# donglinb/ORB-SLAM-BIRDVIEW

Hardware: AMD Instinct MI355X
Metric: ORB features/sec per GPU (1280×720, 2000 kp, 8 levels) + Hamming matches/sec (higher is better)
Workload: dtype u8; 1 GPU; C3 1280x720 KITTI-style synthetic, 2000 features, 8 levels; width=1280, height=720, nfeatures=2000, nlevels=8, ini_th_fast=20, min_th_fast=7, batch_per_gpu=256, global_batch=256, parallelism=frame-sharded x1 (no collective), batches_in_flight=2

## Files before the change

### orb-slam-birdview_amd/csrc/extract_kernels.hip

```cpp
#include "glibc_trig.h"
#include "orbgpu_internal.h"
#include "pattern31_data.inc"

#include <algorithm>
#include <cstring>

namespace orbgpu {

__constant__ __attribute__((aligned(16))) int8_t c_pattern[1024] = {ORBGPU_PATTERN31_VALUES};
__constant__ __attribute__((aligned(16))) float c_pattern_f[1024] = {ORBGPU_PATTERN31_VALUES};

struct IcMaskTable {
    uint32_t m[64][4];
};
constexpr IcMaskTable make_ic_masks() {
    IcMaskTable t{};
    constexpr int umax[16] = {15, 15, 15, 15, 14, 14, 14, 13, 13, 12, 11, 10, 9, 8, 6, 3};
    for (int l = 0; l < 64; l++) {
        const int r = (l >> 1) < 30 ? (l >> 1) : 30, v = r - 15, h = l & 1;
        const int d = umax[v < 0 ? -v : v];
        for (int i = 0; i < 4; i++) {
            uint32_t m = 0;
            for (int j = 0; j < 4; j++) {
                const int u = 4 * (4 * h + i) + j;
// ... 1799 lines not shown
                               err, par, ost);
    else
        octree_level<false, NT, CP>(g, L, f, l, smem, C, keys, knodeAll + o, lvlKps, lvlCount, err, par, ost);
}


template <int NT>
__global__ __launch_bounds__(NT) void k_octree(const Geom* __restrict__ g,
                                                           const uint32_t* __restrict__ cands,
                                                           const uint32_t* __restrict__ candFirst,
                                                           uint32_t* __restrict__ keysAll,
                                                           uint16_t* __restrict__ knodeAll,
                                                           uint32_t* __restrict__ lvlKps, int* __restrict__ lvlCount,
                                                           int* __restrict__ err, int lds_keys,
                                                           unsigned long long* __restrict__ ostamps, int lbase) {
    extern __shared__ __attribute__((aligned(16))) int smem[];
    octree_task<NT, 0>(g, blockIdx.x, lbase + (int)blockIdx.y, smem, cands, candFirst, keysAll, knodeAll, lvlKps,
                       lvlCount, err, lds_keys, ostamps);
}

constexpr float kAtanScale = (float)(180 / 3.14159265358979323846);
constexpr float kP1 = 0.9997878412794807f * kAtanScale;
constexpr float kP3 = -0.3258083974640975f * kAtanScale;
constexpr float kP5 = 0.1555786518463281f * kAtanScale;
constexpr float kP7 = -0.04432655554792128f * kAtanScale;
constexpr float kFactorPI = (float)(3.14159265358979323846 / 180.f);

__device__ __forceinline__ float fast_atan2(float y, float x) {
    const float ax = fabsf(x), ay = fabsf(y);
    float a, c, c2;
    if (ax >= ay) {
        c = ay / (ax + (float)2.220446049250313e-16);
        c2 = c * c;
        a = (((kP7 * c2 + kP5) * c2 + kP3) * c2 + kP1) * c;
    } else {
        c = ax / (ay + (float)2.220446049250313e-16);
        c2 = c * c;
        a = 90.f - (((kP7 * c2 + kP5) * c2 + kP3) * c2 + kP1) * c;
    }
    if (x < 0) a = 180.f - a;
    if (y < 0) a = 360.f - a;
    return a;
}



constexpr int kDescRtCols = 37, kDescWinOff = 2976, kDescWaveBytes = kDescWinOff + kDescWin * kDescWinPitch;
constexpr bool desc_overlap_ok() {
    return 2 * kRtPitch * kDescRtCols <= kDescWinOff + 6 * kDescWinPitch && kDescWinOff % 16 == 0 &&
           kDescWaveBytes % 16 == 0 && 4 * kDescWaveBytes + 256 <= 160 * 1024 / 8;
}
static_assert(desc_overlap_ok(), "k_describe LDS overlap");

struct DescSlot {
    bool ok, interior;
    int s, l, x, y, score, outIdx;
    LevelPtr src;
};

template <int CP = 0>
__device__ __forceinline__ DescSlot desc_slot(const Geom* __restrict__ g, int f, int s, const int* cnts,
                                              const uint32_t* __restrict__ lvlKps, const uint8_t* frames,
                                              long long framePitch, int rowStride, const uint8_t* pyr) {
    DescSlot d;
    d.s = s;
    d.ok = false;
    d.interior = false;
    if (s >= g->nkpcap) return d;
    const int nl = g->nlevels;
    int l = 0;
    while (l + 1 < nl && s >= g->L[l + 1].kp_base) ++l;
    const LevelGeom& L = g->L[l];
    const int k = s - L.kp_base;
    auto cnt = [&](int i) -> int {
        if constexpr (CP != 0) return __hip_atomic_load(&cnts[i], __ATOMIC_RELAXED, __HIP_MEMORY_SCOPE_AGENT);
        else return cnts[i];
    };
    if (k >= cnt(l)) return d;
    int outIdx = k;
    for (int i = 0; i < l; i++) outIdx += cnt(i);
    uint32_t kp;
    if constexpr (CP != 0) kp = __hip_atomic_load(&lvlKps[(long long)f * g->nkpcap + s], __ATOMIC_RELAXED, __HIP_MEMORY_SCOPE_AGENT);
    else kp = lvlKps[(long long)f * g->nkpcap + s];
    d.ok = true;
    d.l = l;
    d.x = kp & 0xFFF;
    d.y = (kp >> 12) & 0xFFF;
    d.score = kp >> 24;
    d.outIdx = outIdx;
    d.src = level_ptr(g, l, frames, framePitch, rowStride, pyr, f);
    const bool aligned = ((reinterpret_cast<uintptr_t>(d.src.p) | (uintptr_t)d.src.stride) & 3) == 0;
    d.interior = aligned && d.x >= 21 && d.x + 27 <= L.w && d.y >= 21 && d.y + 21 < L.h;
    return d;
}

template <int CP = 0>
__device__ __forceinline__ void desc_issue(const DescSlot& d, int lane, uint32_t (&v)[9]) {
    const int a0 = (d.x - 21) & ~3;
    const int stride = __builtin_amdgcn_readfirstlane(d.src.stride);
    const uint64_t rb = reinterpret_cast<uint64_t>(d.src.p + (long long)(d.y - 21) * stride + a0);
    const uint64_t rbu = ((uint64_t)(uint32_t)__builtin_amdgcn_readfirstlane((unsigned)(rb >> 32)) << 32) |
                         (uint64_t)(uint32_t)__builtin_amdgcn_readfirstlane((unsigned)rb);
    const auto rsrc = __builtin_amdgcn_make_buffer_rsrc(reinterpret_cast<void*>(rbu), 0, (kDescWin - 1) * stride + 48,
                                                          0x00020000);
    const int wy0 = (int)(__umul24((unsigned)lane, 2731u) >> 15), ww = lane - wy0 * 12;
    const int off = (int)roi_off(wy0, stride, 4 * ww);
#pragma unroll
    for (int r = 0; r < 8; r++) v[r] = __builtin_amdgcn_raw_buffer_load_b32(rsrc, off, 5 * r * stride, CP);
    v[8] = __builtin_amdgcn_raw_buffer_load_b32(rsrc, lane < 36 ? off : 0x40000000, 40 * stride, CP);
}

template <bool ALLEVEN, bool FMA>
__device__ __forceinline__ void brief_sampled(const uint16_t* rt, float a, float b, const float (&pf)[4][4], int colBase,
                                              int xsimd, ushort2_t K01, ushort2_t K23, ushort2_t K45, ushort2_t K60,
                                              int lane, unsigned long long* __restrict__ dst) {
    typedef const uint32_t __attribute__((address_space(3))) lds_u32;
    constexpr uint32_t kC = (uint32_t)kRtPitch * 0x400000u + 0x4B400000u;
    static_assert((kC & 1u) == 0, "the element bias must keep the parity");
    const uint32_t lbase = (uint32_t)(uintptr_t)(lds_u32*)reinterpret_cast<const uint32_t*>(rt) - 2u * kC;
    const uint32_t xlim = (uint32_t)(xsimd - colBase) + 0x4B400000u;
    const uint32_t bias = sgpr_const(32767u);
    typedef float f32x2_t __attribute__((ext_vector_type(2)));
    const f32x2_t ab = {a, b}, nba = {-b, a}, cr = {12582930.0f, 12582930.0f};
    auto sample = [&](f32x2_t pp) -> uint32_t {
        const f32x2_t pyv = __builtin_shufflevector(pp, pp, 1, 1), pxv = __builtin_shufflevector(pp, pp, 0, 0);
        const f32x2_t t = pyv * nba;
        const f32x2_t r = (FMA ? __builtin_elementwise_fma(pxv, ab, t) : pxv * ab + t) + cr;
        const float fx = r.x, fy = r.y;
        const uint32_t xbits = __builtin_bit_cast(uint32_t, fx);
        const uint32_t ybits = __builtin_bit_cast(uint32_t, fy);
        const uint32_t idx = __umul24(xbits, (unsigned)kRtPitch) + ybits;
        uint32_t ie = idx & ~1u;
        asm("" : "+v"(ie));
        lds_u32* rp = (lds_u32*)(uintptr_t)(lbase + (ie << 1));
        const uint32_t sh = idx << 4;
        const uint32_t d0 = rp[0], d1 = rp[1], d2 = rp[2], d3 = rp[3];
        uint32_t S = __builtin_amdgcn_udot2(K01, __builtin_bit_cast(ushort2_t, __builtin_amdgcn_alignbit(d1, d0, sh)), 0u, false);
        S = __builtin_amdgcn_udot2(K23, __builtin_bit_cast(ushort2_t, __builtin_amdgcn_alignbit(d2, d1, sh)), S, false);
        S = __builtin_amdgcn_udot2(K45, __builtin_bit_cast(ushort2_t, __builtin_amdgcn_alignbit(d3, d2, sh)), S, false);
        S = __builtin_amdgcn_udot2(K60, __builtin_bit_cast(ushort2_t, __builtin_amdgcn_alignbit(d3, d3, sh)), S, false);
        if (ALLEVEN) return S + bias + ((S >> 16) & 1u);
        return S + (xbits < xlim ? bias + ((S >> 16) & 1u) : 32768u);
    };
    unsigned long long mq[4];
#pragma unroll
    for (int gq = 0; gq < 4; gq++) {
        const uint32_t r0 = sample(f32x2_t{pf[gq][0], pf[gq][1]});
        const uint32_t r1 = sample(f32x2_t{pf[gq][2], pf[gq][3]});
        mq[gq] = __ballot((r0 >> 16) < min(r1 >> 16, 255u));
    }
    if (lane < 4) dst[lane] = lane == 0 ? mq[0] : lane == 1 ? mq[1] : lane == 2 ? mq[2] : mq[3];
}

template <bool FMA, int CP = 0>
__device__ __forceinline__ void desc_body(const Geom* __restrict__ g, const DescSlot& d, int f, int lane,
                                          const uint32_t (&v)[9], uint8_t* wbase, uint16_t* rt,
                                          orb_keypoint* __restrict__ outK, uint8_t* __restrict__ outD, int kpCap,
                                          unsigned long long* __restrict__ dstamps) {
    const int l = d.l, x = d.x, y = d.y, score = d.score, outIdx = d.outIdx;
    const LevelGeom& L = g->L[l];
    const LevelPtr src = d.src;
    [[maybe_unused]] unsigned long long* dst_st = dstamps ? dstamps + ((long long)f * g->nkpcap + d.s) * 8 : nullptr;
#if ORBGPU_KERNEL_STAMPS
#define DESC_STAMP(k) \
    if (dst_st && lane == 0) dst_st[(k)] = __builtin_amdgcn_s_memtime();
#else
#define DESC_STAMP(k)
#endif
    DESC_STAMP(0);
    const uint4 mm = reinterpret_cast<const uint4*>(&c_ic_masks.m[0][0])[lane];
    const uint32_t icm[4] = {mm.x, mm.y, mm.z, mm.w};
    uint32_t* w32 = reinterpret_cast<uint32_t*>(wbase);
    int sh;
    if (d.interior) {
#pragma unroll
        for (int r = 0; r < 9; r++)
            if (r < 8 || lane < 36) w32[lane + 60 * r] = v[r];
        sh = (x - 21) & 3;
    } else {
#pragma unroll
        for (int hb = 0; hb < 2; hb++) {
            uint8_t v[15];
#pragma unroll
            for (int r = 0; r < 15; r++) {
                const int idx = lane + 64 * (15 * hb + r);
                const int wy = (int)(__umul24((unsigned)idx, 24386u) >> 20), wx = idx - wy * kDescWin;
                int sy = y - 21 + wy, sx = x - 21 + wx;
                sy = sy < 0 ? -sy : (sy >= L.h ? 2 * L.h - 2 - sy : sy);
                sx = sx < 0 ? -sx : (sx >= L.w ? 2 * L.w - 2 - sx : sx);
                if constexpr (CP != 0) {
                    const auto brs = __builtin_amdgcn_make_buffer_rsrc(const_cast<uint8_t*>(src.p), 0, 0x7FFFFFFF, 0x00020000);
                    v[r] = idx < kDescWin * kDescWin ? __builtin_amdgcn_raw_buffer_load_b8(brs, (int)roi_off(sy, src.stride, sx), 0, CP)
                                                     : (uint8_t)0;
                } else {
                    v[r] = idx < kDescWin * kDescWin ? src.p[roi_off(sy, src.stride, sx)] : (uint8_t)0;
                }
            }
#pragma unroll
            for (int r = 0; r < 15; r++) {
                const int idx = lane + 64 * (15 * hb + r);
                const int wy = (int)(__umul24((unsigned)idx, 24386u) >> 20), wx = idx - wy * kDescWin;
                if (idx < kDescWin * kDescWin) wbase[wy * kDescWinPitch + wx] = v[r];
            }
        }
        sh = 0;
    }
    wave_lds_sync();
    DESC_STAMP(1);
#if defined(ORBGPU_DESC_CUT) && ORBGPU_DESC_CUT == 1
    if (lane == 0) outD[((long long)f * kpCap + outIdx) * 32] = wbase[lane];
    return;
#endif

    int m10 = 0, m01 = 0;
    if (lane < 62) {
        const int v = (lane >> 1) - 15, h = lane & 1;
        const int base = (21 + v) * kDescWinPitch + sh + 6;
        const int d0 = (base >> 2) + 4 * h, bs = base & 3;
        uint32_t w[5];
#pragma unroll
        for (int i = 0; i < 5; i++) w[i] = w32[d0 + i];
        const uint32_t wt0 = 0x04030201u + (uint32_t)h * 0x10101010u;
        uint32_t sI = 0, sW = 0;
#pragma unroll
        for (int i = 0; i < 4; i++) {
            const uint32_t bytes = __builtin_amdgcn_alignbyte(w[i + 1], w[i], bs) & icm[i];
            sI = __builtin_amdgcn_udot4(bytes, 0x01010101u, sI, false);
            sW = __builtin_amdgcn_udot4(bytes, wt0 + (uint32_t)i * 0x04040404u, sW, false);
        }
        m10 = (int)sW - 16 * (int)sI;
        m01 = v * (int)sI;
    }
    m10 = wave_sum(m10);
    m01 = wave_sum(m01);
    const float angle = fast_atan2((float)m01, (float)m10);
    DESC_STAMP(2);
#if defined(ORBGPU_DESC_CUT) && ORBGPU_DESC_CUT == 2
    if (lane == 0) outD[((long long)f * kpCap + outIdx) * 32] = (uint8_t)angle;
    return;
#endif

    {
        typedef int v4i_t __attribute__((ext_vector_type(4)));
        const int4* tp = g->desc_taps + sh * kDescTapTiles * 64 + lane;
        v4i_t bt[kDescTapTiles];
#pragma unroll
        for (int tc = 0; tc < kDescTapTiles; tc++) {
            const int4 q = tp[tc * 64];
            bt[tc] = v4i_t{q.x, q.y, q.z, q.w};
        }
        const int yl = lane & 15, kq = lane >> 4;
        const int bias = 128 * (g->gk[0] + g->gk[1] + g->gk[2] + g->gk[3] + g->gk[4] + g->gk[5] + g->gk[6]);
#pragma unroll
        for (int ty = 0; ty < 3; ty++) {
            const int y = min(16 * ty + yl, kDescWin - 1);
            const uint4 w = *reinterpret_cast<const uint4*>(wbase + y * kDescWinPitch + 16 * kq);
            const v4i_t a = v4i_t{(int)(w.x ^ 0x80808080u), (int)(w.y ^ 0x80808080u), (int)(w.z ^ 0x80808080u),
                                  (int)(w.w ^ 0x80808080u)};
            const int y0 = 16 * ty + 4 * kq;
#pragma unroll
            for (int tc = 0; tc < kDescTapTiles; tc++) {
                v4i_t d = v4i_t{bias, bias, bias, bias};
                d = __builtin_amdgcn_mfma_i32_16x16x64_i8(a, bt[tc], d, 0, 0, 0);
                const int c = 16 * tc + yl;
                if (y0 < kDescWin && c < kDescRtCols) {
                    uint2 pk;
                    pk.x = __builtin_amdgcn_perm((uint32_t)d[1], (uint32_t)d[0], 0x05040100u);
                    pk.y = __builtin_amdgcn_perm((uint32_t)d[3], (uint32_t)d[2], 0x05040100u);
                    *reinterpret_cast<uint2*>(rt + c * kRtPitch + y0) = pk;
                }
            }
        }
    }
    wave_lds_sync();
    DESC_STAMP(3);
#if defined(ORBGPU_DESC_CUT) && ORBGPU_DESC_CUT == 3
    if (lane == 0) outD[((long long)f * kpCap + outIdx) * 32] = (uint8_t)(angle + rt[lane]);
    return;
#endif

    const int xsimd = (g->variant & ORB_VARIANT_BLUR_HALFUP) ? 0 : (L.w & ~3);
    const int k0 = g->gk[0], k1 = g->gk[1], k2 = g->gk[2], k3 = g->gk[3], k4 = g->gk[4], k5 = g->gk[5],
              k6 = g->gk[6];
    const ushort2_t K01 = {(unsigned short)k0, (unsigned short)k1}, K23 = {(unsigned short)k2, (unsigned short)k3},
                    K45 = {(unsigned short)k4, (unsigned short)k5}, K60 = {(unsigned short)k6, 0};
    DESC_STAMP(4);

    float pf[4][4];
#pragma unroll
    for (int gq = 0; gq < 4; gq++) {
        const float4 pp = reinterpret_cast<const float4*>(c_pattern_f)[lane + 64 * gq];
        pf[gq][0] = pp.x;
        pf[gq][1] = pp.y;
        pf[gq][2] = pp.z;
        pf[gq][3] = pp.w;
    }
    const float ang = angle * kFactorPI;
    float a, b;
    glibc_sincosf(ang, &b, &a);
    DESC_STAMP(5);
    unsigned long long* dst = reinterpret_cast<unsigned long long*>(outD + ((long long)f * kpCap + outIdx) * 32);
    if (x + 18 < xsimd) brief_sampled<true, FMA>(rt, a, b, pf, x - 18, xsimd, K01, K23, K45, K60, lane, dst);
    else brief_sampled<false, FMA>(rt, a, b, pf, x - 18, xsimd, K01, K23, K45, K60, lane, dst);
    if (lane == 0) {
        orb_keypoint o;
        o.x = (float)x;
        o.y = (float)y;
        if (l != 0) {
            o.x *= L.scale;
            o.y *= L.scale;
        }
        o.size = L.patch_size;
        o.angle = angle;
        o.response = (float)score;
        o.octave = l;
        o.class_id = -1;
        outK[(long long)f * kpCap + outIdx] = o;
    }
    DESC_STAMP(6);
#undef DESC_STAMP
}

constexpr int kDescWaves = 4, kDescSlotsPerWave = 2;
template <bool FMA>
__global__ __launch_bounds__(256) __attribute__((amdgpu_waves_per_eu(8, 8))) void k_describe(const Geom* __restrict__ g, const uint8_t* __restrict__ frames,
                                                  long long framePitch, int rowStride, const uint8_t* __restrict__ pyr,
                                                  const uint32_t* __restrict__ lvlKps,
                                                  const int* __restrict__ lvlCount, orb_keypoint* __restrict__ outK,
                                                  uint8_t* __restrict__ outD, int* __restrict__ outN, int kpCap,
                                                  unsigned long long* __restrict__ dstamps, int spw,
                                                  const int* __restrict__ err, int* __restrict__ errHost) {
    __shared__ __attribute__((aligned(16))) uint8_t s_desc[kDescWaves * kDescWaveBytes + 256];
    uint8_t* const s_wave = s_desc + (size_t)__builtin_amdgcn_readfirstlane(threadIdx.x >> 6) * kDescWaveBytes;
    const int gx = (g->nkpcap + kDescWaves * spw - 1) / (kDescWaves * spw);
    const int nb = gridDim.x, q = nb >> 3, r = nb & 7, xcd = blockIdx.x & 7, j = blockIdx.x >> 3;
    const int lb = (xcd < r ? xcd * (q + 1) : r * (q + 1) + (xcd - r) * q) + j;
    const int f = lb / gx, bx = lb - f * gx;
    const int wv = __builtin_amdgcn_readfirstlane(threadIdx.x >> 6), lane = threadIdx.x & 63;
    const int nl = g->nlevels;
    const int* cnts = lvlCount + f * nl;
    const int s0 = (bx * kDescWaves + wv) * spw;
    auto write_n = [&]() {
        if (bx == 0 && threadIdx.x == 0) {
            int tot = 0;
            for (int i = 0; i < nl; i++) tot += cnts[i];
            outN[f] = tot;
            if (errHost && f == 0) *errHost = err[0] | err[1];
        }
    };
    if (s0 >= g->nkpcap) {
        write_n();
        return;
    }
    const DescSlot d0 = desc_slot(g, f, s0, cnts, lvlKps, frames, framePitch, rowStride, pyr);
    const DescSlot d1 = spw == 2 ? desc_slot(g, f, s0 + 1, cnts, lvlKps, frames, framePitch, rowStride, pyr)
                                 : DescSlot{};
    if (!d0.ok && !d1.ok) {
        write_n();
        return;
    }
    uint32_t v0[9], v1[9];
    if (d0.ok && d0.interior) desc_issue(d0, lane, v0);
    if (d1.ok && d1.interior) desc_issue(d1, lane, v1);
    write_n();
    if (d0.ok) desc_body<FMA>(g, d0, f, lane, v0, s_wave + kDescWinOff, reinterpret_cast<uint16_t*>(s_wave), outK, outD, kpCap, dstamps);
    if (d1.ok) {
        __builtin_amdgcn_sched_barrier(0);
        wave_lds_sync();
        desc_body<FMA>(g, d1, f, lane, v1, s_wave + kDescWinOff, reinterpret_cast<uint16_t*>(s_wave), outK, outD, kpCap, dstamps);
    }
}

__global__ __launch_bounds__(256) void k_upload_stream(const uint8_t* __restrict__ h_img, const uint32_t* h_flags,
                                                       uint32_t seq, uint8_t* __restrict__ d_img, int pitch, int h,
                                                       int band_rows, uint32_t* __restrict__ err) {
    __shared__ int s_ok;
    const int b = blockIdx.x;
    if (threadIdx.x == 0) {
        int ok = 0;
        for (int it = 0; it < (1 << 22); it++) {
            if (__hip_atomic_load(h_flags + b, __ATOMIC_RELAXED, __HIP_MEMORY_SCOPE_SYSTEM) == seq) {
                ok = 1;
                break;
            }
            __builtin_amdgcn_s_sleep(2);
        }
        if (!ok) *err = 1;
        s_ok = ok;
    }
    __syncthreads();
    if (!s_ok) return;
    __atomic_thread_fence(__ATOMIC_ACQUIRE);
    const int r0 = b * band_rows, r1 = min(h, r0 + band_rows);
    const size_t n16 = (size_t)(r1 - r0) * pitch / 16;
    const uint4* src = reinterpret_cast<const uint4*>(h_img + (size_t)r0 * pitch);
    uint4* dst = reinterpret_cast<uint4*>(d_img + (size_t)r0 * pitch);
    const size_t st = (size_t)gridDim.y * 256;
    for (size_t i = blockIdx.y * 256 + threadIdx.x; i < n16; i += 4 * st) {
        uint4 v[4];
#pragma unroll
        for (int u = 0; u < 4; u++)
            if (i + u * st < n16) v[u] = src[i + u * st];
#pragma unroll
        for (int u = 0; u < 4; u++)
            if (i + u * st < n16) dst[i + u * st] = v[u];
    }
}

hipError_t launch_upload_stream(const uint8_t* h_img, const uint32_t* h_flags, uint32_t seq, uint8_t* d_img, int pitch,
                                int h, int nbands, int band_rows, uint32_t* h_fail, hipStream_t stream) {
    hipLaunchKernelGGL(k_upload_stream, dim3(nbands, 4), dim3(256), 0, stream, h_img, h_flags, seq, d_img, pitch, h,
                       band_rows, h_fail);
    return hipGetLastError();
}

__global__ __launch_bounds__(256) void k_debug_sincosf(const float* __restrict__ x, int n, float* __restrict__ s,
                                                       float* __restrict__ c) {
    const int i = blockIdx.x * 256 + threadIdx.x;
    if (i >= n) return;
    float sv, cv;
    glibc_sincosf(x[i], &sv, &cv);
    s[i] = sv;
    c[i] = cv;
}

hipError_t launch_debug_sincosf(const float* d_x, int n, float* d_s, float* d_c, hipStream_t stream) {
    if (n <= 0) return hipSuccess;
    hipLaunchKernelGGL(k_debug_sincosf, dim3((n + 255) / 256), dim3(256), 0, stream, d_x, n, d_s, d_c);
    return hipGetLastError();
}


__device__ __forceinline__ int flow_ld(const int* p) { return __hip_atomic_load(p, __ATOMIC_RELAXED, __HIP_MEMORY_SCOPE_AGENT); }
__device__ __forceinline__ void flow_st(int* p, int v) { __hip_atomic_store(p, v, __ATOMIC_RELAXED, __HIP_MEMORY_SCOPE_AGENT); }
__device__ __forceinline__ int flow_add(int* p, int v) {
    return __hip_atomic_fetch_add(p, v, __ATOMIC_RELAXED, __HIP_MEMORY_SCOPE_AGENT);
}

template <int TQ>
__device__ __forceinline__ void flow_fast(const FlowArgs* __restrict__ Ap, int l, int f, int a, int b, int wv, int lane,
                                          uint8_t* smem) {
    if (wv >= b) return;
    const Geom* __restrict__ g = Ap->g;
    const int wb = g->fast_wave_bytes;
    uint16_t* tile = reinterpret_cast<uint16_t*>(smem + (size_t)wv * wb + 16);
    uint16_t* sList = reinterpret_cast<uint16_t*>(smem + (size_t)wv * wb + ((g->fast_rows * TQ * 2 + 32 + 15) & ~15));
    const int cell = g->L[l].cell_base + a + wv;
    const FastCellT c = fast_cell_t(g, Ap->cells, f * g->ncells + cell, Ap->frames, Ap->framePitch, Ap->rowStride,
                                    Ap->pyr, 0, g->ncells);
    uint32_t* candFirst = Ap->candFirst;
    int* cntOut = reinterpret_cast<int*>(candFirst + ((long long)c.f * g->ncells + c.cell) * kCandRec);
    if (!c.valid) {
        if (lane == 0) flow_st(cntOut, 0);
        return;
    }
    uint32_t v[8];
    if (c.aligned) fast_roi_issue<kCpSc1>(c, lane, v);
    fast_roi_store<TQ, kCpSc1>(c, lane, v, tile);
    fast_cell_body<TQ, kCpSc1>(g, c, lane, tile, sList, Ap->cands, candFirst, cntOut, nullptr, 0);
}

__device__ __forceinline__ void flow_resize(const FlowArgs* __restrict__ Ap, int l, int f, int a, int b, int tid,
                                            uint8_t* smem) {
    const Geom* __restrict__ g = Ap->g;
    const int q = tid >> 8;
    const int th = (g->L[l].rs_tiled & 2) ? 32 : 16;
    const int gxl = (g->L[l].w + kRsTileW - 1) / kRsTileW;
    const int tile = a + q;
    const int by = tile / gxl, bx = tile - by * gxl;
    const int rq = Ap->rsQuarter;
    uint8_t* qb = smem + (size_t)q * rq;
    int4* scx = reinterpret_cast<int4*>(qb + rq - (kRsTileW + 32) * 16);
    int4* scy = scx + kRsTileW;
    const ResizeCoef* cf = Ap->rcoef + Ap->roff.o[l];
    const bool on = q < b;
    const bool gen = (g->variant & ORB_VARIANT_RESIZE_GENERIC) != 0;
    const uint8_t* frames = Ap->frames;
    const long long fp = Ap->framePitch;
    const int rs = Ap->rowStride;
    uint8_t* pyr = Ap->pyr;
    if (th == 32) {
        if (gen) resize_tile<32, true, kCpSc1>(g, cf, l, frames, fp, rs, pyr, f, bx, by, tid & 255, qb, scx, scy, on);
        else resize_tile<32, false, kCpSc1>(g, cf, l, frames, fp, rs, pyr, f, bx, by, tid & 255, qb, scx, scy, on);
    } else {
        if (gen) resize_tile<16, true, kCpSc1>(g, cf, l, frames, fp, rs, pyr, f, bx, by, tid & 255, qb, scx, scy, on);
        else resize_tile<16, false, kCpSc1>(g, cf, l, frames, fp, rs, pyr, f, bx, by, tid & 255, qb, scx, scy, on);
    }
}

__device__ __forceinline__ void flow_chain(const FlowArgs* __restrict__ Ap, int f, int a, int b, int seg, int tid,
                                           uint8_t* smem) {
    const Geom* __restrict__ g = Ap->g;
    const int q = tid >> 8;
    const int rq = Ap->rsQuarter;
    uint8_t* qb = smem + (size_t)q * rq;
    int4* sreg = reinterpret_cast<int4*>(qb + rq - ORBGPU_MAX_LEVELS * 16);
    const ChainJob* J = Ap->chainJobs + a + (q < b ? q : 0);
    const ChainSegment sg = Ap->chainSeg[seg];
    RcoefOff ro = Ap->roff;
    if (g->variant & ORB_VARIANT_RESIZE_GENERIC)
        chain_job<true, kCpSc1>(g, Ap->rcoef, J, sg, ro, Ap->frames, Ap->framePitch, Ap->rowStride, Ap->pyr, f, tid & 255, qb, sreg);
    else
        chain_job<false, kCpSc1>(g, Ap->rcoef, J, sg, ro, Ap->frames, Ap->framePitch, Ap->rowStride, Ap->pyr, f, tid & 255, qb, sreg);
}

template <bool FMA>
__device__ __forceinline__ void flow_describe(const FlowArgs* __restrict__ Ap, int f, int a, int b, int wv, int lane,
                                              uint8_t* smem) {
    if (wv >= b) return;
    const Geom* __restrict__ g = Ap->g;
    uint8_t* sw = smem + (size_t)wv * kDescWaveBytes;
    const DescSlot d = desc_slot<kCpSc1>(g, f, a + wv, Ap->lvlCount + f * g->nlevels, Ap->lvlKps, Ap->frames,
                                         Ap->framePitch, Ap->rowStride, Ap->pyr);
    if (!d.ok) return;
    uint32_t v[9];
    if (d.interior) desc_issue<kCpSc1>(d, lane, v);
    desc_body<FMA, kCpSc1>(g, d, f, lane, v, sw + kDescWinOff, reinterpret_cast<uint16_t*>(sw), Ap->outK, Ap->outD,
                           Ap->kpCap, nullptr);
}

template <int TQ, bool FMA>
__global__ __launch_bounds__(kFlowThreads) void k_extract_flow(const FlowArgs* __restrict__ Ap0) {
    extern __shared__ __attribute__((aligned(16))) uint8_t fl_smem[];
    __shared__ int s_tk[2];
    if (threadIdx.x == 0) s_tk[0] = flow_add(&Ap0->ctr[0], 1);
    __syncthreads();
    int cur = __builtin_amdgcn_readfirstlane(s_tk[0]);
    while (cur < Ap0->ntasks) {
        int tid;
        asm volatile("v_mov_b32 %0, %1" : "=v"(tid) : "v"((int)threadIdx.x));
        const int lane = tid & 63;
        const int wv = __builtin_amdgcn_readfirstlane(tid >> 6);
        const FlowArgs* __restrict__ Ap = Ap0;
        asm volatile("" : "+s"(Ap));
        const FlowTask t = Ap->tasks[cur];
        const int kind = t.klf & 0xFF, l = (t.klf >> 8) & 0xFF, f = t.klf >> 16;
        unsigned long long* st = Ap->stamps ? Ap->stamps + 4 * (size_t)cur : nullptr;
        if (tid == 0) {
            if (st) st[0] = __builtin_amdgcn_s_memrealtime();
            int* ctr = Ap->ctr;
            s_tk[1] = flow_add(&ctr[0], 1);
            if (t.nd > 0 && !flow_ld(&ctr[48])) {
                const unsigned long long t0 = __builtin_amdgcn_s_memrealtime();
                bool late = false;
                for (int k = 0; k < t.nd && !late; k++)
                    while (flow_ld(&ctr[t.dep + k]) < t.tgt) {
                        __builtin_amdgcn_s_sleep(1);
                        if (__builtin_amdgcn_s_memrealtime() - t0 > 20000000ull || flow_ld(&ctr[48])) {
                            __hip_atomic_fetch_or(&ctr[48], 1, __ATOMIC_RELAXED, __HIP_MEMORY_SCOPE_AGENT);
                            late = true;
                            break;
                        }
                    }
            }
        }
        __syncthreads();
        if (st && tid == 0) st[1] = __builtin_amdgcn_s_memrealtime();
        const int nxt = __builtin_amdgcn_readfirstlane(s_tk[1]);
        if (kind == kFlowChain) {
            flow_chain(Ap, f, t.a, t.b, t.seg, tid, fl_smem);
        } else if (kind == kFlowResize) {
            flow_resize(Ap, l, f, t.a, t.b, tid, fl_smem);
        } else if (kind == kFlowFast) {
            flow_fast<TQ>(Ap, l, f, t.a, t.b, wv, lane, fl_smem);
        } else if (kind == kFlowOctree) {
            const Geom* __restrict__ g = Ap->g;
            const int nl = g->nlevels;
            int* eword = &Ap->ctr[kFlowCtrBase + 4 * nl * f + 3 * nl + l];
            octree_task<kFlowThreads, kCpSc1>(g, f, l, reinterpret_cast<int*>(fl_smem), Ap->cands, Ap->candFirst,
                                              Ap->keys, Ap->knode, Ap->lvlKps, Ap->lvlCount, eword, Ap->ldsKeys, nullptr);
        } else {
            flow_describe<FMA>(Ap, f, t.a, t.b, wv, lane, fl_smem);
        }
        asm volatile("s_waitcnt vmcnt(0)" ::: "memory");
        __syncthreads();
        if (st && tid == 0) {
            st[2] = __builtin_amdgcn_s_memrealtime();
            st[3] = (unsigned long long)(unsigned)t.klf | ((unsigned long long)blockIdx.x << 32);
        }
        if (tid == 0 && t.sig >= 0) {
            int* ctr = Ap->ctr;
            flow_add(&ctr[t.sig], 1);
            const int nl = Ap->g->nlevels, nfr = Ap->nframes;
            if (kind == kFlowOctree && flow_add(&ctr[32], 1) == nfr * nl - 1) {
                int e = 0;
                const int* lc = Ap->lvlCount;
                for (int fr = 0; fr < nfr; fr++) {
                    int tot = 0;
                    for (int i = 0; i < nl; i++) {
                        tot += flow_ld(&lc[fr * nl + i]);
                        e |= flow_ld(&ctr[kFlowCtrBase + 4 * nl * fr + 3 * nl + i]);
                    }
                    Ap->outN[fr] = tot;
                }
                Ap->err[0] = e;
                Ap->err[1] = 0;
                if (Ap->errHost) *Ap->errHost = e;
            }
        }
        cur = nxt;
    }
    if (threadIdx.x == 0) {
        const FlowArgs* __restrict__ Ap = Ap0;
        int* ctr = Ap->ctr;
        if (flow_add(&ctr[16], 1) == (int)gridDim.x - 1) {
            if (flow_ld(&ctr[48])) {
                Ap->err[1] = 4;
                if (Ap->errHost) *Ap->errHost = 4;
            }
            const int n = kFlowCtrBase + 4 * Ap->g->nlevels * Ap->nframes;
            for (int i = 0; i < n; i++) flow_st(&ctr[i], 0);
        }
    }
}

static inline unsigned cdiv(unsigned a, unsigned b) { return (a + b - 1) / b; }

size_t octree_lds_bytes(int node_cap) { return (size_t)node_cap * (16 * 4) + (32 + 8) * 4; }

static int octree_lds_keys(int node_cap) {
    const long long room = 52 * 1024 - (long long)octree_lds_bytes(node_cap);
    return room > 0 ? (int)((room / 6) & ~7LL) : 0;
}
static int octree_lds_keys_whole_cu(const Geom& g) {
    const long long room = 160 * 1024 - (long long)octree_lds_bytes(g.node_cap);
    const long long want = ((long long)g.max_level_cand + 7) & ~7LL;
    return room > 0 ? (int)std::min(want, (room / 6) & ~7LL) : 0;
}

bool build_flow(const Geom& g, int nframes, int blocks, const ChainPlan* chain, const std::vector<ChainJob>* jobs,
                std::vector<FlowTask>& tasks, FlowPlan& plan) {
    tasks.clear();
    plan = FlowPlan{};
    const int nl = g.nlevels;
    if (nframes < 1 || nframes > 0xFFFF) return false;
    const bool chained = chain && jobs && chain->nseg > 0 && chain->first_base == 0;
    int rsq = 0;
    for (int l = 1; l < nl && !chained; l++) {
        if (!(g.L[l].rs_tiled & 3)) return false;
        rsq = std::max(rsq, ((g.L[l].rs_span_rows * kRsPitch + 15) & ~15) + (kRsTileW + 32) * 16);
    }
    if (chained)
        for (int sgi = 0; sgi < chain->nseg; sgi++)
            rsq = std::max(rsq, ((chain->seg[sgi].lds_bytes + 15) & ~15) + ORBGPU_MAX_LEVELS * 16);
    int nres[ORBGPU_MAX_LEVELS] = {0}, nfast[ORBGPU_MAX_LEVELS] = {0};
    for (int l = 0; l < nl; l++) {
        if (l > 0) {
            const int th = (g.L[l].rs_tiled & 2) ? 32 : 16;
            const int tiles = (int)(cdiv(g.L[l].w, kRsTileW) * cdiv(g.L[l].h, th));
            nres[l] = (tiles + 3) / 4;
        }
        nfast[l] = (g.L[l].nCols * g.L[l].nRows + 15) / 16;
    }
    auto ctr = [&](int f, int part, int l) { return kFlowCtrBase + 4 * nl * f + part * nl + l; };
    auto push = [&](int kind, int l, int f, int sig, int a, int b, int dep, int nd, int tgt) {
        FlowTask t;
        t.klf = kind | (l << 8) | (f << 16);
        t.sig = sig;
        t.a = a;
        t.b = b;
        t.dep = dep;
        t.nd = nd;
        t.tgt = tgt;
        t.seg = 0;
        tasks.push_back(t);
    };
    int nchain[ORBGPU_MAX_LEVELS] = {0}, cj0[ORBGPU_MAX_LEVELS] = {0}, cjn[ORBGPU_MAX_LEVELS] = {0},
        cseg[ORBGPU_MAX_LEVELS] = {0}, cbase[ORBGPU_MAX_LEVELS] = {0};
    if (chained) {
        for (int sgi = 0; sgi < chain->nseg; sgi++) {
            const ChainSegment& sg = chain->seg[sgi];
// ... 229 lines not shown
```

Measured before the change: 385.6 million features/s.

## Pair two keypoints per wave to share orientation and trig computation

Splits the descriptor body into helper functions and adds a paired path for waves that own two valid keypoints, the second one interior. Both windows go to LDS at once: the second is parked in the row-table region. Both intensity-centroid moments are computed in one stretch, and one atan2/sincos call serves both keypoints, with lanes 0-31 handling the first and lanes 32-63 the second, after which the results are read back per keypoint. The aim is to remove the serial latency of a second moment and trig pass. The cost is an extra window store and more register pressure.

Measured after the change: 391.3 million features/s, median of 6. 1.01x the previous value.

```diff
diff --git a/orb-slam-birdview_amd/csrc/extract_kernels.hip b/orb-slam-birdview_amd/csrc/extract_kernels.hip
--- a/orb-slam-birdview_amd/csrc/extract_kernels.hip
+++ b/orb-slam-birdview_amd/csrc/extract_kernels.hip
@@ -1975,66 +1975,73 @@
     if (lane < 4) dst[lane] = lane == 0 ? mq[0] : lane == 1 ? mq[1] : lane == 2 ? mq[2] : mq[3];
 }
 
-template <bool FMA, int CP = 0>
-__device__ __forceinline__ void desc_body(const Geom* __restrict__ g, const DescSlot& d, int f, int lane,
-                                          const uint32_t (&v)[9], uint8_t* wbase, uint16_t* rt,
-                                          orb_keypoint* __restrict__ outK, uint8_t* __restrict__ outD, int kpCap,
-                                          unsigned long long* __restrict__ dstamps) {
-    const int l = d.l, x = d.x, y = d.y, score = d.score, outIdx = d.outIdx;
-    const LevelGeom& L = g->L[l];
+
+__device__ __forceinline__ void desc_stamp([[maybe_unused]] unsigned long long* st, [[maybe_unused]] int lane,
+                                           [[maybe_unused]] int k) {
+#if ORBGPU_KERNEL_STAMPS
+    if (st && lane == 0) st[k] = __builtin_amdgcn_s_memtime();
+#endif
+}
+
+__device__ __forceinline__ void desc_ic_masks(int lane, uint32_t (&icm)[4]) {
+    const uint4 mm = reinterpret_cast<const uint4*>(&c_ic_masks.m[0][0])[lane];
+    icm[0] = mm.x;
+    icm[1] = mm.y;
+    icm[2] = mm.z;
+    icm[3] = mm.w;
+}
+
+__device__ __forceinline__ int desc_store_regs(const DescSlot& d, int lane, const uint32_t (&v)[9], uint32_t* w32) {
+#pragma unroll
+    for (int r = 0; r < 9; r++)
+        if (r < 8 || lane < 36) w32[lane + 60 * r] = v[r];
+    return (d.x - 21) & 3;
+}
+
+template <int CP>
+__device__ __forceinline__ int desc_store_gather(const Geom* __restrict__ g, const DescSlot& d, int lane, uint8_t* wbase) {
+    const int x = d.x, y = d.y;
+    const LevelGeom& L = g->L[d.l];
     const LevelPtr src = d.src;
-    [[maybe_unused]] unsigned long long* dst_st = dstamps ? dstamps + ((long long)f * g->nkpcap + d.s) * 8 : nullptr;
-#if ORBGPU_KERNEL_STAMPS
-#define DESC_STAMP(k) \
-    if (dst_st && lane == 0) dst_st[(k)] = __builtin_amdgcn_s_memtime();
-#else
-#define DESC_STAMP(k)
-#endif
-    DESC_STAMP(0);
-    const uint4 mm = reinterpret_cast<const uint4*>(&c_ic_masks.m[0][0])[lane];
-    const uint32_t icm[4] = {mm.x, mm.y, mm.z, mm.w};
-    uint32_t* w32 = reinterpret_cast<uint32_t*>(wbase);
-    int sh;
-    if (d.interior) {
-#pragma unroll
-        for (int r = 0; r < 9; r++)
-            if (r < 8 || lane < 36) w32[lane + 60 * r] = v[r];
-        sh = (x - 21) & 3;
-    } else {
-#pragma unroll
-        for (int hb = 0; hb < 2; hb++) {
-            uint8_t v[15];
-#pragma unroll
-            for (int r = 0; r < 15; r++) {
-                const int idx = lane + 64 * (15 * hb + r);
-                const int wy = (int)(__umul24((unsigned)idx, 24386u) >> 20), wx = idx - wy * kDescWin;
-                int sy = y - 21 + wy, sx = x - 21 + wx;
-                sy = sy < 0 ? -sy : (sy >= L.h ? 2 * L.h - 2 - sy : sy);
-                sx = sx < 0 ? -sx : (sx >= L.w ? 2 * L.w - 2 - sx : sx);
-                if constexpr (CP != 0) {
-                    const auto brs = __builtin_amdgcn_make_buffer_rsrc(const_cast<uint8_t*>(src.p), 0, 0x7FFFFFFF, 0x00020000);
-                    v[r] = idx < kDescWin * kDescWin ? __builtin_amdgcn_raw_buffer_load_b8(brs, (int)roi_off(sy, src.stride, sx), 0, CP)
-                                                     : (uint8_t)0;
-                } else {
-                    v[r] = idx < kDescWin * kDescWin ? src.p[roi_off(sy, src.stride, sx)] : (uint8_t)0;
-                }
-            }
-#pragma unroll
-            for (int r = 0; r < 15; r++) {
-                const int idx = lane + 64 * (15 * hb + r);
-                const int wy = (int)(__umul24((unsigned)idx, 24386u) >> 20), wx = idx - wy * kDescWin;
-                if (idx < kDescWin * kDescWin) wbase[wy * kDescWinPitch + wx] = v[r];
-            }
-        }
-        sh = 0;
-    }
-    wave_lds_sync();
-    DESC_STAMP(1);
-#if defined(ORBGPU_DESC_CUT) && ORBGPU_DESC_CUT == 1
-    if (lane == 0) outD[((long long)f * kpCap + outIdx) * 32] = wbase[lane];
-    return;
-#endif
-
+#pragma unroll
+    for (int hb = 0; hb < 2; hb++) {
+        uint8_t v[15];
+#pragma unroll
+        for (int r = 0; r < 15; r++) {
+            const int idx = lane + 64 * (15 * hb + r);
+            const int wy = (int)(__umul24((unsigned)idx, 24386u) >> 20), wx = idx - wy * kDescWin;
+            int sy = y - 21 + wy, sx = x - 21 + wx;
+            sy = sy < 0 ? -sy : (sy >= L.h ? 2 * L.h - 2 - sy : sy);
+            sx = sx < 0 ? -sx : (sx >= L.w ? 2 * L.w - 2 - sx : sx);
+            if constexpr (CP != 0) {
+                const auto brs = __builtin_amdgcn_make_buffer_rsrc(const_cast<uint8_t*>(src.p), 0, 0x7FFFFFFF, 0x00020000);
+                v[r] = idx < kDescWin * kDescWin ? __builtin_amdgcn_raw_buffer_load_b8(brs, (int)roi_off(sy, src.stride, sx), 0, CP)
+                                                 : (uint8_t)0;
+            } else {
+                v[r] = idx < kDescWin * kDescWin ? src.p[roi_off(sy, src.stride, sx)] : (uint8_t)0;
+            }
+        }
+#pragma unroll
+        for (int r = 0; r < 15; r++) {
+            const int idx = lane + 64 * (15 * hb + r);
+            const int wy = (int)(__umul24((unsigned)idx, 24386u) >> 20), wx = idx - wy * kDescWin;
+            if (idx < kDescWin * kDescWin) wbase[wy * kDescWinPitch + wx] = v[r];
+        }
+    }
+    return 0;
+}
+
+template <int CP>
+__device__ __forceinline__ int desc_store_window(const Geom* __restrict__ g, const DescSlot& d, int lane,
+                                                 const uint32_t (&v)[9], uint8_t* wbase) {
+    if (d.interior) return desc_store_regs(d, lane, v, reinterpret_cast<uint32_t*>(wbase));
+    return desc_store_gather<CP>(g, d, lane, wbase);
+}
+
+struct IcMoments {
+    int m01, m10;
+};
+__device__ __forceinline__ IcMoments desc_ic_moments(const uint32_t* w32, int sh, int lane, const uint32_t (&icm)[4]) {
     int m10 = 0, m01 = 0;
     if (lane < 62) {
         const int v = (lane >> 1) - 15, h = lane & 1;
@@ -2054,62 +2061,61 @@
         m10 = (int)sW - 16 * (int)sI;
         m01 = v * (int)sI;
     }
-    m10 = wave_sum(m10);
-    m01 = wave_sum(m01);
-    const float angle = fast_atan2((float)m01, (float)m10);
-    DESC_STAMP(2);
-#if defined(ORBGPU_DESC_CUT) && ORBGPU_DESC_CUT == 2
-    if (lane == 0) outD[((long long)f * kpCap + outIdx) * 32] = (uint8_t)angle;
-    return;
-#endif
-
-    {
-        typedef int v4i_t __attribute__((ext_vector_type(4)));
-        const int4* tp = g->desc_taps + sh * kDescTapTiles * 64 + lane;
-        v4i_t bt[kDescTapTiles];
+    IcMoments m;
+    m.m10 = wave_sum(m10);
+    m.m01 = wave_sum(m01);
+    return m;
+}
+
+__device__ __forceinline__ float desc_trig_angle(float m01, float m10) { return fast_atan2(m01, m10); }
+__device__ __forceinline__ void desc_trig_rotation(float angle, float* a, float* b) {
+    glibc_sincosf(angle * kFactorPI, b, a);
+}
+struct DescTrig {
+    float angle, a, b;
+};
+__device__ __forceinline__ DescTrig desc_trig(float m01, float m10) {
+    DescTrig t;
+    t.angle = desc_trig_angle(m01, m10);
+    desc_trig_rotation(t.angle, &t.a, &t.b);
+    return t;
+}
+
+__device__ __forceinline__ void desc_row_pass(const Geom* __restrict__ g, int sh, int lane, const uint8_t* wbase,
+                                              uint16_t* rt) {
+    typedef int v4i_t __attribute__((ext_vector_type(4)));
+    const int4* tp = g->desc_taps + sh * kDescTapTiles * 64 + lane;
+    v4i_t bt[kDescTapTiles];
+#pragma unroll
+    for (int tc = 0; tc < kDescTapTiles; tc++) {
+        const int4 q = tp[tc * 64];
+        bt[tc] = v4i_t{q.x, q.y, q.z, q.w};
+    }
+    const int yl = lane & 15, kq = lane >> 4;
+    const int bias = 128 * (g->gk[0] + g->gk[1] + g->gk[2] + g->gk[3] + g->gk[4] + g->gk[5] + g->gk[6]);
+#pragma unroll
+    for (int ty = 0; ty < 3; ty++) {
+        const int y = min(16 * ty + yl, kDescWin - 1);
+        const uint4 w = *reinterpret_cast<const uint4*>(wbase + y * kDescWinPitch + 16 * kq);
+        const v4i_t a = v4i_t{(int)(w.x ^ 0x80808080u), (int)(w.y ^ 0x80808080u), (int)(w.z ^ 0x80808080u),
+                              (int)(w.w ^ 0x80808080u)};
+        const int y0 = 16 * ty + 4 * kq;
 #pragma unroll
         for (int tc = 0; tc < kDescTapTiles; tc++) {
-            const int4 q = tp[tc * 64];
-            bt[tc] = v4i_t{q.x, q.y, q.z, q.w};
-        }
-        const int yl = lane & 15, kq = lane >> 4;
-        const int bias = 128 * (g->gk[0] + g->gk[1] + g->gk[2] + g->gk[3] + g->gk[4] + g->gk[5] + g->gk[6]);
-#pragma unroll
-        for (int ty = 0; ty < 3; ty++) {
-            const int y = min(16 * ty + yl, kDescWin - 1);
-            const uint4 w = *reinterpret_cast<const uint4*>(wbase + y * kDescWinPitch + 16 * kq);
-            const v4i_t a = v4i_t{(int)(w.x ^ 0x80808080u), (int)(w.y ^ 0x80808080u), (int)(w.z ^ 0x80808080u),
-                                  (int)(w.w ^ 0x80808080u)};
-            const int y0 = 16 * ty + 4 * kq;
-#pragma unroll
-            for (int tc = 0; tc < kDescTapTiles; tc++) {
-                v4i_t d = v4i_t{bias, bias, bias, bias};
-                d = __builtin_amdgcn_mfma_i32_16x16x64_i8(a, bt[tc], d, 0, 0, 0);
-                const int c = 16 * tc + yl;
-                if (y0 < kDescWin && c < kDescRtCols) {
-                    uint2 pk;
-                    pk.x = __builtin_amdgcn_perm((uint32_t)d[1], (uint32_t)d[0], 0x05040100u);
-                    pk.y = __builtin_amdgcn_perm((uint32_t)d[3], (uint32_t)d[2], 0x05040100u);
-                    *reinterpret_cast<uint2*>(rt + c * kRtPitch + y0) = pk;
-                }
-            }
-        }
-    }
-    wave_lds_sync();
-    DESC_STAMP(3);
-#if defined(ORBGPU_DESC_CUT) && ORBGPU_DESC_CUT == 3
-    if (lane == 0) outD[((long long)f * kpCap + outIdx) * 32] = (uint8_t)(angle + rt[lane]);
-    return;
-#endif
-
-    const int xsimd = (g->variant & ORB_VARIANT_BLUR_HALFUP) ? 0 : (L.w & ~3);
-    const int k0 = g->gk[0], k1 = g->gk[1], k2 = g->gk[2], k3 = g->gk[3], k4 = g->gk[4], k5 = g->gk[5],
-              k6 = g->gk[6];
-    const ushort2_t K01 = {(unsigned short)k0, (unsigned short)k1}, K23 = {(unsigned short)k2, (unsigned short)k3},
-                    K45 = {(unsigned short)k4, (unsigned short)k5}, K60 = {(unsigned short)k6, 0};
-    DESC_STAMP(4);
-
-    float pf[4][4];
+            v4i_t d = v4i_t{bias, bias, bias, bias};
+            d = __builtin_amdgcn_mfma_i32_16x16x64_i8(a, bt[tc], d, 0, 0, 0);
+            const int c = 16 * tc + yl;
+            if (y0 < kDescWin && c < kDescRtCols) {
+                uint2 pk;
+                pk.x = __builtin_amdgcn_perm((uint32_t)d[1], (uint32_t)d[0], 0x05040100u);
+                pk.y = __builtin_amdgcn_perm((uint32_t)d[3], (uint32_t)d[2], 0x05040100u);
+                *reinterpret_cast<uint2*>(rt + c * kRtPitch + y0) = pk;
+            }
+        }
+    }
+}
+
+__device__ __forceinline__ void desc_pattern(int lane, float (&pf)[4][4]) {
 #pragma unroll
     for (int gq = 0; gq < 4; gq++) {
         const float4 pp = reinterpret_cast<const float4*>(c_pattern_f)[lane + 64 * gq];
@@ -2118,13 +2124,34 @@
         pf[gq][2] = pp.z;
         pf[gq][3] = pp.w;
     }
-    const float ang = angle * kFactorPI;
-    float a, b;
-    glibc_sincosf(ang, &b, &a);
-    DESC_STAMP(5);
-    unsigned long long* dst = reinterpret_cast<unsigned long long*>(outD + ((long long)f * kpCap + outIdx) * 32);
-    if (x + 18 < xsimd) brief_sampled<true, FMA>(rt, a, b, pf, x - 18, xsimd, K01, K23, K45, K60, lane, dst);
-    else brief_sampled<false, FMA>(rt, a, b, pf, x - 18, xsimd, K01, K23, K45, K60, lane, dst);
+}
+
+struct DescBlurK {
+    int xsimd;
+    ushort2_t K01, K23, K45, K60;
+};
+__device__ __forceinline__ DescBlurK desc_blur_k(const Geom* __restrict__ g, const DescSlot& d) {
+    DescBlurK k;
+    k.xsimd = (g->variant & ORB_VARIANT_BLUR_HALFUP) ? 0 : (g->L[d.l].w & ~3);
+    const int k0 = g->gk[0], k1 = g->gk[1], k2 = g->gk[2], k3 = g->gk[3], k4 = g->gk[4], k5 = g->gk[5],
+              k6 = g->gk[6];
+    k.K01 = ushort2_t{(unsigned short)k0, (unsigned short)k1};
+    k.K23 = ushort2_t{(unsigned short)k2, (unsigned short)k3};
+    k.K45 = ushort2_t{(unsigned short)k4, (unsigned short)k5};
+    k.K60 = ushort2_t{(unsigned short)k6, 0};
+    return k;
+}
+
+template <bool FMA>
+__device__ __forceinline__ void desc_brief_store(const Geom* __restrict__ g, const DescSlot& d, int f, int lane,
+                                                 const uint16_t* rt, const DescBlurK& k, const float (&pf)[4][4],
+                                                 float angle, float a, float b, orb_keypoint* __restrict__ outK,
+                                                 uint8_t* __restrict__ outD, int kpCap) {
+    const int l = d.l, x = d.x, y = d.y;
+    const LevelGeom& L = g->L[l];
+    unsigned long long* dst = reinterpret_cast<unsigned long long*>(outD + ((long long)f * kpCap + d.outIdx) * 32);
+    if (x + 18 < k.xsimd) brief_sampled<true, FMA>(rt, a, b, pf, x - 18, k.xsimd, k.K01, k.K23, k.K45, k.K60, lane, dst);
+    else brief_sampled<false, FMA>(rt, a, b, pf, x - 18, k.xsimd, k.K01, k.K23, k.K45, k.K60, lane, dst);
     if (lane == 0) {
         orb_keypoint o;
         o.x = (float)x;
@@ -2135,13 +2162,118 @@
         }
         o.size = L.patch_size;
         o.angle = angle;
-        o.response = (float)score;
+        o.response = (float)d.score;
         o.octave = l;
         o.class_id = -1;
-        outK[(long long)f * kpCap + outIdx] = o;
-    }
-    DESC_STAMP(6);
-#undef DESC_STAMP
+        outK[(long long)f * kpCap + d.outIdx] = o;
+    }
+}
+
+__device__ __forceinline__ unsigned long long* desc_stamp_row(const Geom* __restrict__ g, const DescSlot& d, int f,
+                                                              unsigned long long* __restrict__ dstamps) {
+    return dstamps ? dstamps + ((long long)f * g->nkpcap + d.s) * 8 : nullptr;
+}
+
+template <bool FMA, int CP = 0>
+__device__ __forceinline__ void desc_single(const Geom* __restrict__ g, const DescSlot& d, int f, int lane,
+                                            const uint32_t (&v)[9], uint8_t* wbase, uint16_t* rt,
+                                            orb_keypoint* __restrict__ outK, uint8_t* __restrict__ outD, int kpCap,
+                                            unsigned long long* __restrict__ dstamps) {
+    [[maybe_unused]] unsigned long long* st = desc_stamp_row(g, d, f, dstamps);
+    desc_stamp(st, lane, 0);
+    uint32_t icm[4];
+    desc_ic_masks(lane, icm);
+    const int sh = desc_store_window<CP>(g, d, lane, v, wbase);
+    wave_lds_sync();
+    desc_stamp(st, lane, 1);
+#if defined(ORBGPU_DESC_CUT) && ORBGPU_DESC_CUT == 1
+    if (lane == 0) outD[((long long)f * kpCap + d.outIdx) * 32] = wbase[lane];
+    return;
+#endif
+    const IcMoments m = desc_ic_moments(reinterpret_cast<const uint32_t*>(wbase), sh, lane, icm);
+    const float angle = desc_trig_angle((float)m.m01, (float)m.m10);
+    desc_stamp(st, lane, 2);
+#if defined(ORBGPU_DESC_CUT) && ORBGPU_DESC_CUT == 2
+    if (lane == 0) outD[((long long)f * kpCap + d.outIdx) * 32] = (uint8_t)angle;
+    return;
+#endif
+    desc_row_pass(g, sh, lane, wbase, rt);
+    wave_lds_sync();
+    desc_stamp(st, lane, 3);
+#if defined(ORBGPU_DESC_CUT) && ORBGPU_DESC_CUT == 3
+    if (lane == 0) outD[((long long)f * kpCap + d.outIdx) * 32] = (uint8_t)(angle + rt[lane]);
+    return;
+#endif
+    const DescBlurK k = desc_blur_k(g, d);
+    desc_stamp(st, lane, 4);
+    float pf[4][4];
+    desc_pattern(lane, pf);
+    float a, b;
+    desc_trig_rotation(angle, &a, &b);
+    desc_stamp(st, lane, 5);
+    desc_brief_store<FMA>(g, d, f, lane, rt, k, pf, angle, a, b, outK, outD, kpCap);
+    desc_stamp(st, lane, 6);
+}
+
+static_assert(kDescWin * kDescWinPitch <= kDescWinOff, "k_describe: the paired slot's temporary window");
+
+template <bool FMA>
+__device__ __forceinline__ void desc_pair(const Geom* __restrict__ g, const DescSlot& d0, const DescSlot& d1, int f,
+                                          int lane, const uint32_t (&v0)[9], const uint32_t (&v1)[9], uint8_t* wbase,
+                                          uint16_t* rt, orb_keypoint* __restrict__ outK, uint8_t* __restrict__ outD,
+                                          int kpCap, unsigned long long* __restrict__ dstamps) {
+    [[maybe_unused]] unsigned long long* st0 = desc_stamp_row(g, d0, f, dstamps);
+    [[maybe_unused]] unsigned long long* st1 = desc_stamp_row(g, d1, f, dstamps);
+    desc_stamp(st0, lane, 0);
+    uint32_t icm[4];
+    desc_ic_masks(lane, icm);
+    uint32_t* const w32 = reinterpret_cast<uint32_t*>(wbase);
+    uint32_t* const t32 = reinterpret_cast<uint32_t*>(rt);
+    const int sh0 = desc_store_window<0>(g, d0, lane, v0, wbase);
+    const int sh1 = desc_store_regs(d1, lane, v1, t32);
+    wave_lds_sync();
+    desc_stamp(st0, lane, 1);
+    const IcMoments m0 = desc_ic_moments(w32, sh0, lane, icm);
+    const IcMoments m1 = desc_ic_moments(t32, sh1, lane, icm);
+    const bool hi = lane >= 32;
+    const DescTrig t = desc_trig((float)(hi ? m1.m01 : m0.m01), (float)(hi ? m1.m10 : m0.m10));
+    auto lane_f = [](float x, int l) {
+        return __builtin_bit_cast(float, __builtin_amdgcn_readlane(__builtin_bit_cast(int, x), l));
+    };
+    const float angle0 = lane_f(t.angle, 0), a0 = lane_f(t.a, 0), b0 = lane_f(t.b, 0);
+    const float angle1 = lane_f(t.angle, 32), a1 = lane_f(t.a, 32), b1 = lane_f(t.b, 32);
+    desc_stamp(st0, lane, 2);
+    {
+        desc_row_pass(g, sh0, lane, wbase, rt);
+        wave_lds_sync();
+        desc_stamp(st0, lane, 3);
+        const DescBlurK k = desc_blur_k(g, d0);
+        desc_stamp(st0, lane, 4);
+        float pf[4][4];
+        desc_pattern(lane, pf);
+        desc_stamp(st0, lane, 5);
+        desc_brief_store<FMA>(g, d0, f, lane, rt, k, pf, angle0, a0, b0, outK, outD, kpCap);
+        desc_stamp(st0, lane, 6);
+    }
+    __builtin_amdgcn_sched_barrier(0);
+    wave_lds_sync();
+    {
+        desc_stamp(st1, lane, 0);
+        desc_store_regs(d1, lane, v1, w32);
+        wave_lds_sync();
+        desc_stamp(st1, lane, 1);
+        desc_stamp(st1, lane, 2);
+        desc_row_pass(g, sh1, lane, wbase, rt);
+        wave_lds_sync();
+        desc_stamp(st1, lane, 3);
+        const DescBlurK k = desc_blur_k(g, d1);
+        desc_stamp(st1, lane, 4);
+        float pf[4][4];
+        desc_pattern(lane, pf);
+        desc_stamp(st1, lane, 5);
+        desc_brief_store<FMA>(g, d1, f, lane, rt, k, pf, angle1, a1, b1, outK, outD, kpCap);
+        desc_stamp(st1, lane, 6);
+    }
 }
 
 constexpr int kDescWaves = 4, kDescSlotsPerWave = 2;
@@ -2186,11 +2318,22 @@
     if (d0.ok && d0.interior) desc_issue(d0, lane, v0);
     if (d1.ok && d1.interior) desc_issue(d1, lane, v1);
     write_n();
-    if (d0.ok) desc_body<FMA>(g, d0, f, lane, v0, s_wave + kDescWinOff, reinterpret_cast<uint16_t*>(s_wave), outK, outD, kpCap, dstamps);
+    uint8_t* const wbase = s_wave + kDescWinOff;
+    uint16_t* const rt = reinterpret_cast<uint16_t*>(s_wave);
+#ifdef ORBGPU_DESC_CUT
+    constexpr bool kPair = false;
+#else
+    constexpr bool kPair = true;
+#endif
+    if (kPair && d0.ok && d1.ok && d1.interior) {
+        desc_pair<FMA>(g, d0, d1, f, lane, v0, v1, wbase, rt, outK, outD, kpCap, dstamps);
+        return;
+    }
+    if (d0.ok) desc_single<FMA>(g, d0, f, lane, v0, wbase, rt, outK, outD, kpCap, dstamps);
     if (d1.ok) {
         __builtin_amdgcn_sched_barrier(0);
         wave_lds_sync();
-        desc_body<FMA>(g, d1, f, lane, v1, s_wave + kDescWinOff, reinterpret_cast<uint16_t*>(s_wave), outK, outD, kpCap, dstamps);
+        desc_single<FMA>(g, d1, f, lane, v1, wbase, rt, outK, outD, kpCap, dstamps);
     }
 }
 
@@ -2338,8 +2481,8 @@
     if (!d.ok) return;
     uint32_t v[9];
     if (d.interior) desc_issue<kCpSc1>(d, lane, v);
-    desc_body<FMA, kCpSc1>(g, d, f, lane, v, sw + kDescWinOff, reinterpret_cast<uint16_t*>(sw), Ap->outK, Ap->outD,
-                           Ap->kpCap, nullptr);
+    desc_single<FMA, kCpSc1>(g, d, f, lane, v, sw + kDescWinOff, reinterpret_cast<uint16_t*>(sw), Ap->outK, Ap->outD,
+                             Ap->kpCap, nullptr);
 }
 
 template <int TQ, bool FMA>
```
